# rayanirban/DiffSplitting

Measured on AMD Instinct MI355X. Metric: sampled images/sec (2000-step 128x128 SR3), higher is better.
Workload: dtype bf16; 1 GPU; sr_sr3_16_128: GaussianDiffusion.p_sample_loop, 16->128 SR3 UNet (97.8M params), T=2000 linear schedule; one step = UNet forward + posterior update of the batch; batch_per_gpu=16, global_batch=16, image=128x128x3, sample_steps=2000, parallelism=1 independent replicas, final RCCL all-gather, hipgraph=True, streams=1, noise=device Philox4x32-10, weights=random-init, seed 0

## Files before the change

### diffsplitting_amd/csrc/dsx_conv.hip

```cpp
#include "dsx_kernels.h"
#include <algorithm>
#include <cstdlib>
#include <mutex>
#include <type_traits>
#include <utility>

#ifndef DSX_WS_DEPTH_EXPR
#define DSX_WS_DEPTH_EXPR (bm == 64 ? 5 : (bm == 256 ? 2 : (ks == 1 ? 3 : 4)))
#endif
#ifndef DSX_PRE_RESID_EXPR
#define DSX_PRE_RESID_EXPR (NB == 1 && MB <= 2)
#endif
#ifndef DSX_PFF_EXPR
#define DSX_PFF_EXPR (NB == 2 ? 3 : 6)
#endif
#ifndef DSX_WS_K0_EXPR
#define DSX_WS_K0_EXPR 64
#endif
#ifndef DSX_EPI_PRIO_COND
#define DSX_EPI_PRIO_COND false
#endif
#ifndef DSX_STAMP_CVT_COND
#define DSX_STAMP_CVT_COND (tiC == 2 && gC == 0)
#endif
// ... 899 lines not shown
#pragma unroll
      for (int q = 0; q < 2 * NA; ++q) asm volatile("" : "+v"(av[q]));
#pragma unroll
      for (int it = 0; it < NIT; ++it) asm volatile("" : "+v"(rv[it]));
      DSX_STAMP_T(121, tid == 256 && DSX_STAMP_CVT_COND);
      float sc[CPU], sh[CPU];
#pragma unroll
      for (int q = 0; q < NA; ++q) {
        sc[4 * q] = gnF ? av[q].x : 1.0f; sc[4 * q + 1] = gnF ? av[q].y : 1.0f;
        sc[4 * q + 2] = gnF ? av[q].z : 1.0f; sc[4 * q + 3] = gnF ? av[q].w : 1.0f;
        sh[4 * q] = gnF ? av[NA + q].x : 0.0f; sh[4 * q + 1] = gnF ? av[NA + q].y : 0.0f;
        sh[4 * q + 2] = gnF ? av[NA + q].z : 0.0f; sh[4 * q + 3] = gnF ? av[NA + q].w : 0.0f;
      }
      const bool any_gn = a.gn_scale != nullptr;
      const bool plain = KS == 1 && !(gnF || a.swish);
      if (plain) {
#pragma unroll
        for (int it = 0; it < NIT; ++it) {
          if (loff[it] >= 0) {
            uint4 w = __builtin_bit_cast(uint4, rv[it]);
            const unsigned keep = ((edge[it] & flagsF) == 0 && cF < C) ? 0xffffffffu : 0u;
            w.x &= keep; w.y &= keep; w.z &= keep; w.w &= keep;
            lds_write_b128_asm(dst + loff[it], __builtin_bit_cast(f32x4_t, w));
          }
        }
      } else {
#pragma unroll
        for (int it = 0; it < NIT; ++it) {
          if (loff[it] >= 0) {
            float v[CPU];
            Unit<DT>::unpack(__builtin_bit_cast(uint4, rv[it]), v);
#ifndef DSX_ABL_CVT
            if (any_gn) affine_vec(v, sc, sh);
            if (a.swish) swish_vec(v);
#endif
            if (it == NIT - 1) { asm volatile("" :: "v"(v[0]), "v"(v[CPU - 1])); DSX_STAMP_T(122, tid == 256 && DSX_STAMP_CVT_COND); }
            uint4 w = Unit<DT>::pack(v);
            const unsigned keep = ((edge[it] & flagsF) == 0 && cF < C) ? 0xffffffffu : 0u;
            w.x &= keep; w.y &= keep; w.z &= keep; w.w &= keep;
            lds_write_b128_asm(dst + loff[it], __builtin_bit_cast(f32x4_t, w));
          }
        }
      }
      DSX_STAMP_T(123, tid == 256 && DSX_STAMP_CVT_COND);
    };
    auto wait_young = [&](int young) __attribute__((always_inline)) {
      if (young >= P) wait_vmcnt<P * NIT>();
      else if (P > 1 && young == P - 1) wait_vmcnt<(P > 1 ? (P - 1) * NIT : 0)>();
      else if (P > 2 && young == P - 2) wait_vmcnt<(P > 2 ? (P - 2) * NIT : 0)>();
      else if (P > 3 && young == P - 3) wait_vmcnt<(P > 3 ? (P - 3) * NIT : 0)>();
      else wait_vmcnt<0>();
      __builtin_amdgcn_sched_barrier(0);
    };

    int issued = 0, slotI = 0, slotF = 0;
    auto issue_next = [&]() __attribute__((always_inline)) {
      issue(slotI);
      ++issued;
      if (++slotI == NSLOT) slotI = 0;
    };
    auto fetch_next = [&]() __attribute__((always_inline)) {
      fetch(slotF);
      if (++slotF == NSLOT) slotF = 0;
    };
    DSX_STAMP_T(110, tid == 256);
    constexpr int K0 = DSX_WS_K0_EXPR < NSLOT ? DSX_WS_K0_EXPR : NSLOT;
    while (issued < K0 && issued < total) issue_next();
    DSX_STAMP_T(111, tid == 256);
    ws_barrier();
    wait_young(issued - 1);
    DSX_STAMP_T(112, tid == 256);
    fetch_next();
    for (int k = 0; k < 2 && issued < total && issued < NSLOT; ++k) issue_next();
    convert(0);
    if constexpr (NBUF >= 3) { if (total > 0) lds_signal(full_addr, wave, 1); }
    DSX_STAMP_T(113, tid == 256);
    if (total > 1) {
      wait_young(issued - 2);
      fetch_next();
    }
    if constexpr (NBUF == 2) ws_barrier();
    DSX_STAMP_T(64, tid == 256);
    int bufL = 1;
    for (int v = 0; v < total; ++v) {
      for (int k = 0; k < 2 && issued < total && issued < v + 1 + NSLOT; ++k) issue_next();
      DSX_STAMP_T(65 + 4 * v, tid == 256 && v < 9);
      if (v + 1 < total) {
        if constexpr (NBUF >= 3) {
          if (v + 1 >= NBUF) lds_wait_all_ge(full_addr + 16, v + 2 - NBUF, a.handoff_timeouts);
          convert(bufL);
          lds_signal(full_addr, wave, v + 2);
        } else {
          convert((v + 1) & 1);
        }
      }
      if (++bufL == NBUF) bufL = 0;
      DSX_STAMP_T(66 + 4 * v, tid == 256 && v < 9);
      if (v + 2 < total) {
        wait_young(issued - (v + 3));
        fetch_next();
      }
      DSX_STAMP_T(67 + 4 * v, tid == 256 && v < 9);
      if constexpr (NBUF == 2) ws_barrier();
      DSX_STAMP_T(68 + 4 * v, tid == 256 && v < 9);
    }
    return;
  }

  const int wm = wave / WN, wn = wave % WN;
  const int pq = ws16_pixel(c16);
  int abase[MB][KS];
#pragma unroll
  for (int mb = 0; mb < MB; ++mb) {
    const int m = (wm * MB + mb) * 32 + pq;
    const int tx = m & (TW - 1);
    const int ty = (m >> a.tw_log2) & (TH - 1);
    const int tb = m >> (a.tw_log2 + a.th_log2);
#pragma unroll
    for (int dy = 0; dy < KS; ++dy)
      abase[mb][dy] = (tb * PH + ty * S + dy) * RB + tx * S * PIXB + ws16_slice(kq) * 16;
  }
  const int a16 = TW >= 32 ? 16 * S * PIXB : (16 >> a.tw_log2) * S * RB;
  const int blk0 = (nt * WN + wn) * NB;
  const int wblock = G * (NSTEP * 1024);
  const __amdgpu_buffer_rsrc_t rsw = __builtin_amdgcn_make_buffer_rsrc(
      (void*)((const unsigned char*)a.wpack + (size_t)blk0 * wblock), 0, NB * wblock, 0x00020000);
  const int wlane[2] = {ws16_woff(lane, 0), ws16_woff(lane, 1)};
  static_assert(D % 2 == 0 && NSTEP % 2 == 0, "ring slots alternate between the two fragments of a pair");
  const int qtot = G * NSTEP;
  int qn = 0;
  struct WFrag { uint4 v[NB]; };
  auto load_b = [&](auto chc) __attribute__((always_inline)) -> WFrag {
    constexpr int ch = decltype(chc)::value;
    WFrag f;
#pragma unroll
    for (int nb = 0; nb < NB; ++nb)
      f.v[nb] = __builtin_bit_cast(uint4, __builtin_amdgcn_raw_buffer_load_b128(rsw, wlane[ch], nb * wblock + (qn >> 1) * 2048, 0));
    if (++qn == qtot) qn = 0;
    return f;
  };
  WFrag bq[D];
  static_for<D>([&](auto jc) __attribute__((always_inline)) {
    bq[decltype(jc)::value] = load_b(std::integral_constant<int, (decltype(jc)::value & 1)>{});
  });

  f32x16 acc[MB][NB];
#pragma unroll
  for (int mb = 0; mb < MB; ++mb)
#pragma unroll
    for (int nb = 0; nb < NB; ++nb)
#pragma unroll
      for (int r = 0; r < 16; ++r) acc[mb][nb][r] = 0.0f;

  const bool do_stats = a.stat_part != nullptr;
  const int nbase = blk0 * 32 + 8 * kq;

  struct TilePos { int tx, ty, b; };
  const int per_img = a.tiles_x * a.tiles_y;
  const int adv_x = a.ws_adv_x, adv_y = a.ws_adv_y, adv_b = a.ws_adv_b;
  auto tile_advance = [&](TilePos& t) __attribute__((always_inline)) {
    t.tx += adv_x;
    if (t.tx >= a.tiles_x) { t.tx -= a.tiles_x; t.ty += 1; }
    t.ty += adv_y;
    if (t.ty >= a.tiles_y) { t.ty -= a.tiles_y; t.b += 1; }
    t.b += adv_b;
  };
  int orow[MB], rrow[MB];
#pragma unroll
  for (int mb = 0; mb < MB; ++mb) {
    const int m = (wm * MB + mb) * 32 + pq;
    const int pix = (m >> a.tw_log2) * a.Wo + (m & (TW - 1));
    orow[mb] = pix * a.out_ld + nbase;
    rrow[mb] = pix * a.resid_ld + nbase;
  }
  const int p16 = TW >= 32 ? 16 : (16 >> a.tw_log2) * a.Wo;
  const int o16 = p16 * a.out_ld, r16 = p16 * a.resid_ld;
  auto tile_pixel0 = [&](const TilePos& t) __attribute__((always_inline)) -> int {
    return (t.b * a.Ho + (t.ty << a.th_log2)) * a.Wo + (t.tx << a.tw_log2);
  };
  TilePos cur;
  {
    const int q1 = (int)fastdiv((unsigned)p0, a.mg_tiles_x);
    cur.b = (int)fastdiv((unsigned)p0, a.mg_per_img);
    cur.tx = p0 - q1 * a.tiles_x;
    cur.ty = q1 - cur.b * a.tiles_y;
  }
  TilePos nxt = cur;
  tile_advance(nxt);
  TilePos nn = nxt;
  tile_advance(nn);

  auto load_aff = [&](int b, int slot) __attribute__((always_inline)) {
    if (a.gn_scale == nullptr || tid * 4 >= C) return;
    float* dst = aff_base + (size_t)slot * (AFFB / 4);
    *(float4*)(dst + tid * 4) = *(const float4*)(a.gn_scale + (size_t)b * C + tid * 4);
    *(float4*)(dst + C + tid * 4) = *(const float4*)(a.gn_shift + (size_t)b * C + tid * 4);
  };
  TilePos n3 = nn;
  tile_advance(n3);
  load_aff(cur.b, 0);
  if (ntile > 1) load_aff(nxt.b, 1);
  if (ntile > 2) load_aff(nn.b, 2);

  constexpr int NR = 8 / CPU;
  const float4 zero4 = make_float4(0.f, 0.f, 0.f, 0.f);
  float4 addv[NB][2], affv[2];
  constexpr bool PRE_RESID = DSX_PRE_RESID_EXPR;
  uint4 residv[PRE_RESID ? MB : 1][NB][2][NR];
#pragma unroll
  for (int nb = 0; nb < NB; ++nb)
#pragma unroll
    for (int j = 0; j < 2; ++j) addv[nb][j] = zero4;
  if (a.bias && !a.film) {
#pragma unroll
    for (int nb = 0; nb < NB; ++nb)
#pragma unroll
      for (int j = 0; j < 2; ++j) addv[nb][j] = *(const float4*)(a.bias + nbase + 32 * nb + 4 * j);
  }
#pragma unroll
  for (int mb = 0; mb < (PRE_RESID ? MB : 1); ++mb)
#pragma unroll
    for (int nb = 0; nb < NB; ++nb)
#pragma unroll
      for (int ph = 0; ph < 2; ++ph)
#pragma unroll
        for (int q = 0; q < NR; ++q) residv[mb][nb][ph][q] = make_uint4(0u, 0u, 0u, 0u);
  affv[0] = affv[1] = zero4;
  auto prefetch_epilogue = [&](const TilePos& t, bool want_aff, int b_aff) __attribute__((always_inline)) {
    if (a.film) {
#pragma unroll
      for (int nb = 0; nb < NB; ++nb)
#pragma unroll
        for (int j = 0; j < 2; ++j)
          addv[nb][j] = *(const float4*)(a.film + (size_t)t.b * a.film_bs + nbase + 32 * nb + 4 * j);
    }
    if (PRE_RESID && a.resid) {
      const int r0 = tile_pixel0(t) * a.resid_ld;
#pragma unroll
      for (int mb = 0; mb < (PRE_RESID ? MB : 1); ++mb)
#pragma unroll
        for (int ph = 0; ph < 2; ++ph) {
          const DT* rp = (const DT*)a.resid + (r0 + rrow[mb] + ph * r16);
#pragma unroll
          for (int nb = 0; nb < NB; ++nb)
#pragma unroll
            for (int q = 0; q < NR; ++q) residv[mb][nb][ph][q] = *(const uint4*)(rp + 32 * nb + CPU * q);
        }
    }
    if (want_aff && a.gn_scale != nullptr && tid * 4 < C) {
      affv[0] = *(const float4*)(a.gn_scale + (size_t)b_aff * C + tid * 4);
      affv[1] = *(const float4*)(a.gn_shift + (size_t)b_aff * C + tid * 4);
    }
  };
  prefetch_epilogue(cur, ntile > 3, n3.b);

  constexpr bool PF_OK = !(NB == 2 && KS == 3);
  unsigned fin_pf_acc = 0u;
  if constexpr (PF_OK) fin_pf_acc = l2_prefetch_fold(l2_prefetch(a.pf, blockIdx.x, gridDim.x, tid, 256));
  if constexpr (KS == 1) {
    if (a.fin_on) {
      fin_pf_acc |= l2_prefetch_fold(l2_prefetch(a.fin.pf, blockIdx.x, gridDim.x, tid, 256));
      const int nitems = a.fin.B * a.fin.groups;
      for (int item = (int)blockIdx.x * 4 + wave; item < nitems; item += (int)gridDim.x * 4)
        gn_finalize_item<1>(a.fin, item % a.fin.B, item / a.fin.B, lane, nullptr);
    }
  }

  if constexpr (NBUF >= 3) {
    if (tid < 8) ((unsigned*)(lds + NBUF * BUFB + 3 * AFFB + NSLOT * RAWB))[tid] = 0u;
  }
  ws_barrier();
  if constexpr (NBUF == 2) ws_barrier();
  DSX_STAMP_T(0, tid == 0);
  int g = 0, ti = 0, aslot = 0;
  int ibuf = 0;
  constexpr int NPAIR = NSTEP / 2;
  constexpr int NF = 2 * MB;
  constexpr int FT = NPAIR * NF;
  constexpr int PFF = (DSX_PFF_EXPR) < FT ? (DSX_PFF_EXPR) : FT - 1;
  static_assert(PFF >= 1 && PFF < FT && PFF <= 15, "lgkmcnt is 4 bits");
  constexpr int RP = D > NSTEP ? D / NSTEP : 1;
  if constexpr (RP == 1) {
    for (int v = 0; v < total; ++v) {
      constexpr int R0 = 0;
#define DSX_WS_ITEM_NEXT continue
#include "dsx_conv_ws_item.inc"
#undef DSX_WS_ITEM_NEXT
    }
  } else {
    for (int v0 = 0; v0 < total; v0 += RP)
      static_for<RP>([&](auto rc_) __attribute__((always_inline)) {
        constexpr int R0 = decltype(rc_)::value * NSTEP;
        const int v = v0 + decltype(rc_)::value;
        if (v >= total) return;
#define DSX_WS_ITEM_NEXT return
#include "dsx_conv_ws_item.inc"
#undef DSX_WS_ITEM_NEXT
      });
  }
  if constexpr (PF_OK) l2_prefetch_retire(a.pf, fin_pf_acc);
}


template <typename DT, int KS, int NPH>
__global__ __launch_bounds__(512, 1) void k_conv_img(const ConvArgs a) {
  constexpr int KC = Chunk<DT>::KC;
  constexpr int CPU = Unit<DT>::N;
  constexpr int ES = (int)sizeof(DT);
  constexpr int TAPS = KS * KS, PAD = KS / 2, PW = 8 + 2 * PAD;
  constexpr int PIXB = 80;
  constexpr int RB = KS == 3 ? 896 : 640;
  constexpr int IMGB = PW * RB;
  constexpr int NSTEP = TAPS * 2;
  constexpr int D = NSTEP;
  constexpr int MAXP = NPH;
  constexpr bool ALLW = NPH == 2;
  static_assert(NSTEP % D == 0, "ring depth divides the steps of a phase");
  extern __shared__ __attribute__((aligned(16))) unsigned char lds[];

  const int tid = threadIdx.x, lane = tid & 63;
  const int wave = __builtin_amdgcn_readfirstlane(tid >> 6);
  const int li = lane & 31, lh = lane >> 5;
  const int nb = blockIdx.x % a.nblocks, b = blockIdx.x / a.nblocks;
  const int C = a.C0 + a.C1;
  const int nphase = NPH != 8 ? NPH : C / (8 * KC);
  unsigned char* img = lds + wave * (2 * IMGB);
  float* aff = (float*)(lds + 8 * 2 * IMGB) + wave * (8 * 2 * KC);

  DSX_STAMP(0);
  if (KS == 3) {
    for (int q = lane; q < 360; q += 64) {
      const int bufi = q >= 180, r = q - 180 * bufi, bp = r / 5, u = r - 5 * bp;
      int py, px2;
      if (bp < 10) { py = 0; px2 = bp; }
      else if (bp < 20) { py = 9; px2 = bp - 10; }
      else { py = 1 + ((bp - 20) >> 1); px2 = ((bp - 20) & 1) ? 9 : 0; }
      *(uint4*)(img + bufi * IMGB + py * RB + px2 * PIXB + u * 16) = make_uint4(0u, 0u, 0u, 0u);
    }
  }

  auto load_raw = [&](int p, uint4 (&raw)[4]) __attribute__((always_inline)) {
    const int c0 = (p * 8 + wave) * KC;
    const bool first = c0 < a.C0;
    const char* src = (const char*)(first ? a.src0 : a.src1);
    const int Cs = first ? a.C0 : a.C1, cl = first ? c0 : c0 - a.C0;
#pragma unroll
    for (int i = 0; i < 4; ++i) {
      const int q = lane + 64 * i, px = q >> 2, u = q & 3;
      raw[i] = *(const uint4*)(src + (((size_t)b * 64 + px) * Cs + cl + u * CPU) * ES);
    }
  };
  auto convert_store = [&](int p, const uint4 (&raw)[4]) __attribute__((always_inline)) {
    unsigned char* buf = img + (p & 1) * IMGB;
    const int u = lane & 3;
    float sc[CPU], sh[CPU];
    if (a.has_gn) {
#pragma unroll
      for (int j = 0; j < CPU; ++j) { sc[j] = aff[p * 2 * KC + u * CPU + j]; sh[j] = aff[p * 2 * KC + KC + u * CPU + j]; }
    }
#pragma unroll
    for (int i = 0; i < 4; ++i) {
      const int px = (lane + 64 * i) >> 2;
      float v[CPU];
      Unit<DT>::unpack(raw[i], v);
      if (a.has_gn) affine_vec(v, sc, sh);
      if (a.swish) swish_vec(v);
      *(uint4*)(buf + ((px >> 3) + PAD) * RB + ((px & 7) + PAD) * PIXB + u * 16) = Unit<DT>::pack(v);
    }
  };

  uint2 glo[MAXP], ghi[MAXP];
  float gg[MAXP], gb[MAXP];
  if (a.has_gn) {
#pragma unroll
    for (int p = 0; p < MAXP; ++p) {
      const int pp = p < nphase ? p : nphase - 1;
      const int c0 = (pp * 8 + wave) * KC, cb = c0 & ~63, c = cb + lane;
      const bool first = cb < a.C0;
      const char* part = (const char*)(first ? a.gn_part0 : a.gn_part1);
      const int nch = first ? a.gn_nchunk0 : a.gn_nchunk1, pf32 = first ? a.gn_pf32_0 : a.gn_pf32_1;
      const int Cs = first ? a.C0 : a.C1, cl = first ? c : c - a.C0;
      const char* e = part + (((size_t)b * nch) * Cs + cl) * (pf32 ? 8 : 16);
      glo[p] = *(const uint2*)e;
      ghi[p] = *(const uint2*)(e + 8);
      gg[p] = a.gn_gamma[c]; gb[p] = a.gn_beta[c];
    }
  }
  uint4 raw0[4], raw1[4];
  load_raw(0, raw0);
  if (nphase > 1) load_raw(1, raw1);

  const unsigned char* wbase = (const unsigned char*)a.wpack + (size_t)nb * a.kchunks * (NSTEP * 1024) + lane * 16;
  int pn = 0, sn = 0;
  auto load_w = [&]() __attribute__((always_inline)) -> uint4 {
    const uint4 v = *(const uint4*)(wbase + ((size_t)(pn * 8 + wave) * NSTEP + sn) * 1024);
    if (++sn == NSTEP) { sn = 0; ++pn; }
    return v;
  };
  uint4 wq[D], wq1[ALLW ? D : 1];
#pragma unroll
  for (int j = 0; j < D; ++j) wq[j] = load_w();
  if constexpr (ALLW) {
    if (nphase > 1) {
#pragma unroll
      for (int j = 0; j < D; ++j) wq1[j] = load_w();
    }
  }
  DSX_STAMP(1);

  if (a.has_gn) {
    const int cpg = C / a.gn_groups;
    double gs[MAXP], gq[MAXP];
#pragma unroll
    for (int p = 0; p < MAXP; ++p) {
      const int pp = p < nphase ? p : nphase - 1;
      const int cb = ((pp * 8 + wave) * KC) & ~63, c = cb + lane;
      const bool first = cb < a.C0;
      const int nch = first ? a.gn_nchunk0 : a.gn_nchunk1, pf32 = first ? a.gn_pf32_0 : a.gn_pf32_1;
      const double d0 = __builtin_bit_cast(double, ((unsigned long long)glo[p].y << 32) | glo[p].x);
      const double d1 = __builtin_bit_cast(double, ((unsigned long long)ghi[p].y << 32) | ghi[p].x);
      gs[p] = pf32 ? (double)__builtin_bit_cast(float, glo[p].x) : d0;
      gq[p] = pf32 ? (double)__builtin_bit_cast(float, glo[p].y) : d1;
      if (nch > 1 && p < nphase) {
        const char* part = (const char*)(first ? a.gn_part0 : a.gn_part1);
        const int Cs = first ? a.C0 : a.C1, cl = first ? c : c - a.C0;
        for (int k = 1; k < nch; ++k) {
          const size_t idx = (((size_t)b * nch + k) * Cs + cl) * 2;
          if (pf32) { const float2 v = *(const float2*)((const float*)part + idx); gs[p] += v.x; gq[p] += v.y; }
          else { const double2 v = *(const double2*)((const double*)part + idx); gs[p] += v.x; gq[p] += v.y; }
        }
      }
      const StatPivot& piv = first ? a.gn_piv0 : a.gn_piv1;
      if (piv.bias || piv.film)
        stat_unshift(gs[p], gq[p], (double)stat_pivot(piv, b, first ? c : c - a.C0), (double)(a.Hs * a.Ws));
    }
    const float inv_n = 1.0f / (64.0f * (float)cpg);
#pragma unroll
    for (int p = 0; p < MAXP; ++p) {
      if (p < nphase) {
        const int c0 = (p * 8 + wave) * KC, c = (c0 & ~63) + lane;
        float s = (float)gs[p], q = (float)gq[p];
        for (int o = 1; o < cpg; o <<= 1) { s += __shfl_xor(s, o, 64); q += __shfl_xor(q, o, 64); }
        const double mean = (double)s * (double)inv_n;
        double var = (double)q * (double)inv_n - mean * mean;
        if (var < 0) var = 0;
        const float rstd = __builtin_amdgcn_rsqf((float)var + a.gn_eps);
        const float meanf = (float)mean;
        if (c >= c0 && c < c0 + KC) {
          const float sc = rstd * gg[p];
          aff[p * 2 * KC + (c - c0)] = sc;
          aff[p * 2 * KC + KC + (c - c0)] = gb[p] - meanf * sc;
        }
      }
    }
  }
  const PfAcc pf_acc = l2_prefetch(a.pf, blockIdx.x, gridDim.x, tid, 512);
  DSX_STAMP(2);
  __builtin_amdgcn_s_waitcnt(0xC07F);
  convert_store(0, raw0);
  if (nphase > 1) convert_store(1, raw1);
  DSX_STAMP(3);

  int abase[2][KS];
#pragma unroll
  for (int mb = 0; mb < 2; ++mb) {
    const int m = mb * 32 + li;
#pragma unroll
    for (int dy = 0; dy < KS; ++dy) abase[mb][dy] = ((m >> 3) + dy) * RB + (m & 7) * PIXB + lh * 16;
  }
  f32x16 acc[2];
#pragma unroll
  for (int mb = 0; mb < 2; ++mb)
#pragma unroll
    for (int r = 0; r < 16; ++r) acc[mb][r] = 0.f;

  for (int p = 0; p < nphase; ++p) {
    const unsigned char* buf = img + (p & 1) * IMGB;
    if (p + 2 < nphase) load_raw(p + 2, raw0);
    const bool more = p + 1 < nphase;
    static_for<NSTEP>([&](auto sc_) __attribute__((always_inline)) {
      constexpr int s = decltype(sc_)::value;
      constexpr int tap = s >> 1, fs = s & 1, dy = tap / KS, dx = tap % KS;
      uint4 wcur = wq[s % D];
      if constexpr (ALLW) {
        if (p == 1) wcur = wq1[s % D];
      } else {
        if (more) wq[s % D] = load_w();
      }
#pragma unroll
      for (int mb = 0; mb < 2; ++mb) {
        const f32x4_t px = *(const f32x4_t*)(buf + abase[mb][dy] + dx * PIXB + fs * 32);
        acc[mb] = mfma_step<DT>(wcur, px, acc[mb]);
      }
    });
    if (p + 2 < nphase) convert_store(p + 2, raw0);
    DSX_STAMP(4 + p);
  }

  const int px = tid >> 3, cg = (tid & 7) * 4;
  const int n0 = nb * 32 + cg;
  const size_t opix = (size_t)b * 64 + px;
  float4 eb = make_float4(0.f, 0.f, 0.f, 0.f), ef = eb;
  float er[4] = {0.f, 0.f, 0.f, 0.f};
  if (a.bias) eb = *(const float4*)(a.bias + n0);
  if (a.film) ef = *(const float4*)(a.film + (size_t)b * a.film_bs + n0);
  if (a.resid) {
#pragma unroll
    for (int j = 0; j < 4; ++j) er[j] = act_load<DT>(a.resid, opix * a.resid_ld + n0 + j);
  }
  __syncthreads();
  DSX_STAMP(12);
  float* part = (float*)lds;
#pragma unroll
  for (int mb = 0; mb < 2; ++mb)
#pragma unroll
    for (int j = 0; j < 4; ++j)
      *(float4*)(part + ((wave * 2 + mb) * 64 + lane) * 20 + 4 * j) =
          make_float4(acc[mb][4 * j], acc[mb][4 * j + 1], acc[mb][4 * j + 2], acc[mb][4 * j + 3]);
  __syncthreads();
  DSX_STAMP(13);
  const int mbo = px >> 5, lo = (px & 31) + 32 * (cg >> 4), r0 = cg & 15;
  float x[4] = {0.f, 0.f, 0.f, 0.f};
#pragma unroll
  for (int w = 0; w < 8; ++w) {
    const float4 t = *(const float4*)(part + ((w * 2 + mbo) * 64 + lo) * 20 + r0);
    x[0] += t.x; x[1] += t.y; x[2] += t.z; x[3] += t.w;
  }
  x[0] += eb.x; x[1] += eb.y; x[2] += eb.z; x[3] += eb.w;
  x[0] += ef.x; x[1] += ef.y; x[2] += ef.z; x[3] += ef.w;
#pragma unroll
  for (int j = 0; j < 4; ++j) x[j] += er[j];
  const int okind = a.out_bf16;
  if (okind == 0) {
    *(float4*)((float*)a.out + opix * a.out_ld + n0) = make_float4(x[0], x[1], x[2], x[3]);
  } else {
    uint2 w2;
    if (okind == 1) { w2.x = pack_bf16x2(x[0], x[1]); w2.y = pack_bf16x2(x[2], x[3]); }
    else { w2.x = pack_f16x2(x[0], x[1]); w2.y = pack_f16x2(x[2], x[3]); }
    *(uint2*)((unsigned short*)a.out + opix * a.out_ld + n0) = w2;
  }
  DSX_STAMP(14);
  if (a.stat_part != nullptr) {
    float s1[4], s2[4];
#pragma unroll
    for (int j = 0; j < 4; ++j) { s1[j] = x[j]; s2[j] = x[j] * x[j]; }
#pragma unroll
    for (int o = 8; o < 64; o <<= 1)
#pragma unroll
      for (int j = 0; j < 4; ++j) { s1[j] += __shfl_xor(s1[j], o, 64); s2[j] += __shfl_xor(s2[j], o, 64); }
    __syncthreads();
    float* red = (float*)lds;
    if (lane < 8) {
#pragma unroll
      for (int j = 0; j < 4; ++j) { red[(wave * 32 + cg + j) * 2] = s1[j]; red[(wave * 32 + cg + j) * 2 + 1] = s2[j]; }
    }
    __syncthreads();
    if (tid < 64) {
      const int ch = tid >> 1, k = tid & 1;
      float t = 0.f;
#pragma unroll
      for (int w = 0; w < 8; ++w) t += red[(w * 32 + ch) * 2 + k];
      a.stat_part[((size_t)b * a.Cout + nb * 32 + ch) * 2 + k] = t;
    }
  }
  l2_prefetch_retire(a.pf, pf_acc);
  DSX_STAMP(15);
}

static size_t conv_img_lds(int dtype, int ks) {
  const int KC = dtype != 0 ? 32 : 16;
  const int pw = ks == 3 ? 10 : 8, rb = ks == 3 ? 896 : 640;
  return (size_t)8 * 2 * pw * rb + (size_t)8 * 8 * 2 * KC * sizeof(float);
}
bool conv_img_applicable(int dtype, int ks, int stride, const ConvArgs& a, bool gn, int gn_groups) {
  if (stride != 1 || a.up || !(ks == 1 || ks == 3)) return false;
  if (a.Hs != 8 || a.Ws != 8 || a.Ho != 8 || a.Wo != 8) return false;
  const int KC = dtype != 0 ? 32 : 16, C = a.C0 + a.C1;
  if (a.C0 % (8 * KC) || a.C1 % (8 * KC) || C / (8 * KC) > 8 || C < 8 * KC) return false;
  if (a.Cout % 32 || (a.out_ld & 3) || (a.resid && (a.resid_ld & 3))) return false;
  if (gn) {
    if (gn_groups < 1 || C % gn_groups) return false;
    const int cpg = C / gn_groups;
    if (cpg > 64 || (cpg & (cpg - 1)) || a.C0 % cpg) return false;
  }
  return true;
}


template <typename DT>
__global__ __launch_bounds__(256) void k_conv_first(const ConvArgs a) {
  constexpr bool F32 = sizeof(DT) == 4;
  constexpr int ES = (int)sizeof(DT);
  constexpr int KSTEP = F32 ? 2 : 16;
  constexpr int NS16 = 4;
  __shared__ __attribute__((aligned(16))) unsigned char sm[18 * 18 * 7 * 4 + 64 * 4];
  DT* patch = (DT*)sm;
  int* kofft = (int*)(sm + 18 * 18 * 7 * 4);

  const int tid = threadIdx.x, lane = tid & 63;
  const int wave = __builtin_amdgcn_readfirstlane(tid >> 6);
  const int li = lane & 31, lh = lane >> 5;
  const int Cin = a.C0 + a.C1, K = 9 * Cin;
  const int tiles_x = a.Wo >> 4, tiles_y = a.Ho >> 4;
  const int t = blockIdx.x % (tiles_x * tiles_y), b = blockIdx.x / (tiles_x * tiles_y);
  const int ty = t / tiles_x, tx = t - ty * tiles_x;
  const int oy0 = ty * 16, ox0 = tx * 16;
  const int NBLK = (a.Cout + 31) >> 5;

  for (int e = tid; e < 18 * 18 * Cin; e += 256) {
    const int c = e % Cin, pp = e / Cin, px = pp % 18, py = pp / 18;
    const int iy = oy0 + py - 1, ix = ox0 + px - 1;
    DT v = (DT)0.f;
    if (iy >= 0 && iy < a.Hs && ix >= 0 && ix < a.Ws) {
      const size_t pix = ((size_t)b * a.Hs + iy) * a.Ws + ix;
      v = c < a.C0 ? ((const DT*)a.src0)[pix * a.C0 + c] : ((const DT*)a.src1)[pix * a.C1 + (c - a.C0)];
    }
    patch[e] = v;
  }
  if (F32 && tid < 64) {
    const int k = tid < K ? tid : 0;
    const int tap = k / Cin, c = k - tap * Cin;
    kofft[tid] = ((tap / 3) * 18 + (tap % 3)) * Cin + c;
  }
  int koff[F32 ? 1 : NS16 * 8];
  if constexpr (!F32) {
#pragma unroll
    for (int s = 0; s < NS16; ++s)
#pragma unroll
      for (int j = 0; j < 8; ++j) {
        int k = 16 * s + 8 * lh + j;
        if (k >= K) k = 0;
        const int tap = k / Cin, c = k - tap * Cin;
        koff[s * 8 + j] = (((tap / 3) * 18 + (tap % 3)) * Cin + c) * 2;
      }
  }
  uint4 wf[F32 ? 1 : 2 * NS16];
  if constexpr (!F32) {
#pragma unroll
    for (int nb = 0; nb < 2; ++nb)
#pragma unroll
      for (int s = 0; s < NS16; ++s)
        wf[nb * NS16 + s] = nb < NBLK ? ((const uint4*)a.wpack)[(nb * NS16 + s) * 64 + lane] : make_uint4(0u, 0u, 0u, 0u);
  }
  __syncthreads();

  f32x16 acc[2][2];
#pragma unroll
  for (int mb = 0; mb < 2; ++mb)
#pragma unroll
    for (int nb = 0; nb < 2; ++nb)
#pragma unroll
      for (int r = 0; r < 16; ++r) acc[mb][nb][r] = 0.f;

#pragma unroll
  for (int mb = 0; mb < 2; ++mb) {
    const int m = (wave * 2 + mb) * 32 + li;
    const int base = ((m >> 4) * 18 + (m & 15)) * Cin;
    if constexpr (F32) {
      const int nsteps = (K + 1) >> 1;
      const float* wp = (const float*)a.wpack;
      for (int s = 0; s < nsteps; ++s) {
        const float pv = ((const float*)patch)[base + kofft[2 * s + lh]];
#pragma unroll
        for (int nb = 0; nb < 2; ++nb) {
          if (nb < NBLK) acc[mb][nb] = __builtin_amdgcn_mfma_f32_32x32x2f32(wp[(nb * 32 + s) * 64 + lane], pv, acc[mb][nb], 0, 0, 0);
        }
      }
    } else {
      const unsigned char* pb = (const unsigned char*)patch + base * 2;
#pragma unroll
      for (int s = 0; s < NS16; ++s) {
        unsigned w4[4];
#pragma unroll
        for (int q = 0; q < 4; ++q) {
          const unsigned lo = *(const unsigned short*)(pb + koff[s * 8 + 2 * q]);
          const unsigned hi = *(const unsigned short*)(pb + koff[s * 8 + 2 * q + 1]);
          w4[q] = lo | (hi << 16);
        }
        const f32x4_t px = __builtin_bit_cast(f32x4_t, make_uint4(w4[0], w4[1], w4[2], w4[3]));
#pragma unroll
        for (int nb = 0; nb < 2; ++nb)
          if (nb < NBLK) acc[mb][nb] = mfma_step<DT>(wf[nb * NS16 + s], px, acc[mb][nb]);
      }
    }
  }
  (void)KSTEP; (void)ES;

  const int okind = a.out_bf16;
#pragma unroll
  for (int nb = 0; nb < 2; ++nb) {
    const int nbase = nb * 32 + 16 * lh;
    if (nb >= NBLK) continue;
    float s1[16], s2[16];
#pragma unroll
    for (int r = 0; r < 16; ++r) { s1[r] = 0.f; s2[r] = 0.f; }
    const bool live = nbase < a.Cout;
#pragma unroll
    for (int mb = 0; mb < 2; ++mb) {
      const int m = (wave * 2 + mb) * 32 + li;
      const size_t opix = ((size_t)b * a.Ho + (oy0 + (m >> 4))) * a.Wo + (ox0 + (m & 15));
      float x[16], pv[16];
#pragma unroll
      for (int r = 0; r < 16; ++r) { x[r] = acc[mb][nb][r]; pv[r] = 0.f; }
      if (live) {
        if (a.bias) {
#pragma unroll
          for (int j = 0; j < 4; ++j) { const float4 tt = *(const float4*)(a.bias + nbase + 4 * j); pv[4 * j] = tt.x; pv[4 * j + 1] = tt.y; pv[4 * j + 2] = tt.z; pv[4 * j + 3] = tt.w; }
#pragma unroll
          for (int r = 0; r < 16; ++r) x[r] += pv[r];
        }
        store16<true>(a.out, opix * a.out_ld + nbase, x, okind, 16);
#pragma unroll
        for (int r = 0; r < 16; ++r) { const float d = x[r] - pv[r]; s1[r] += d; s2[r] += d * d; }
      }
    }
    if (a.stat_part != nullptr) {
      float w1 = row16_fold(s1, lane), w2 = row16_fold(s2, lane);
      w1 += __shfl_xor(w1, 16, 64);
      w2 += __shfl_xor(w2, 16, 64);
      const int nch = tiles_x * tiles_y * 4, chunk = t * 4 + wave;
      const int n = nbase + row16_fold_reg(li);
      if (li < 16 && n < a.Cout) {
        float* pp = a.stat_part + (((size_t)b * nch + chunk) * a.Cout + n) * 2;
        pp[0] = w1; pp[1] = w2;
      }
    }
  }
}

bool conv_first_applicable(int ks, int stride, const ConvArgs& a, bool gn) {
  const int C = a.C0 + a.C1;
  return ks == 3 && stride == 1 && !a.up && !gn && !a.swish && C >= 1 && C <= 7 && a.Cout >= 16 && a.Cout <= 64 &&
         (a.Cout & 15) == 0 && (a.Ho & 15) == 0 && (a.Wo & 15) == 0 && a.Ho == a.Hs && a.Wo == a.Ws && a.out_ld == a.Cout;
}
hipError_t launch_conv_first(int dtype, const ConvArgs& a, hipStream_t st) {
  const unsigned grid = (unsigned)(a.B * (a.Ho >> 4) * (a.Wo >> 4));
  if (dtype == 1) hipLaunchKernelGGL(k_conv_first<__bf16>, dim3(grid), dim3(256), 0, st, a);
  else if (dtype == 2) hipLaunchKernelGGL(k_conv_first<_Float16>, dim3(grid), dim3(256), 0, st, a);
  else hipLaunchKernelGGL(k_conv_first<float>, dim3(grid), dim3(256), 0, st, a);
  return hipGetLastError();
}

enum ConvFamily { FAM_MFMA, FAM_WS, FAM_IMG };
struct ConvVariant {
  int family, dtype, tile, ks, stride, cpg;
  void (*kern)(const ConvArgs);
  int block, lds_cap;
  int MB, WM, WN, NB;
  int max_px;
  int nit;
  int depth, nbuf;
  bool fuses_stats;
};
static constexpr int kLdsDefault = 64 * 1024, kLdsMax = 160 * 1024;
static constexpr int conv_cpg(int ks) { return ks == 1 ? 2 : 1; }
int conv_chunk_multiple(int ks) { return conv_cpg(ks); }

static constexpr int mfma_max_px(int bm, int ks, int stride, int cpg) {
  if (ks == 1) return bm;
  if (stride == 2) return 400;
  if (cpg == 2) return bm == 256 ? 324 : 220;
  return bm == 256 ? 400 : (bm == 128 ? 220 : 144);
}
template <typename DT, int TILE, int MB, int WM, int WN, int KS, int S = 1, int CPG = conv_cpg(KS)>
constexpr ConvVariant mfma_row() {
  constexpr bool G2 = KS == 3 && CPG == 2;
  constexpr int D = KS == 1 ? 4 : (G2 ? 6 : DSX_RING_DEPTH);
  constexpr int PX = mfma_max_px(32 * MB * WM, KS, S, CPG);
  constexpr int MI = (PX * 4 * CPG + 255) / 256;
  return {FAM_MFMA, Kind<DT>::value, TILE, KS, S, CPG, k_conv_mfma<DT, MB, WM, WN, KS, S, CPG, D, MI>, 256,
          G2 ? kLdsMax : kLdsDefault, MB, WM, WN, 1, PX, MI, 0, 2, MB <= 2};
}

static constexpr int kWsLoaderWaves = 4;
static constexpr int ws_max_px(int bm, int ks) { return ks == 1 ? bm : (bm == 256 ? 324 : (bm == 128 ? 180 : 108)); }
static constexpr int ws_depth(int bm, int ks, int cpg) {
#ifndef DSX_WS_DEPTH_C2_64
#define DSX_WS_DEPTH_C2_64 3
#endif
  if (ks == 3 && cpg == 2) return bm == 64 ? DSX_WS_DEPTH_C2_64 : 2;
  if (ks == 3 && cpg == 4) return 1;
  if (ks == 1 && cpg == 4) return bm == 64 ? 2 : 1;
  return DSX_WS_DEPTH_EXPR;
}
template <typename DT, int TILE, int MB, int WM, int WN, int NB, int KS, int CPG = conv_cpg(KS)>
constexpr ConvVariant ws_row() {
  constexpr int BM = 32 * MB * WM;
  constexpr int D = KS == 1 ? ((NB == 2 || MB == 4) ? DSX_RING_1X1_NB2 : DSX_RING_1X1_NB1) : ((NB == 2 || MB == 4) ? 6 : 18);
  constexpr int PX = ws_max_px(BM, KS);
  constexpr int NIT = (PX * 4 * CPG + kWsLoaderWaves * 64 - 1) / (kWsLoaderWaves * 64);
  constexpr int P = ws_depth(BM, KS, CPG);
  return {FAM_WS, Kind<DT>::value, TILE, KS, 1, CPG, k_conv_ws<DT, MB, WM, WN, NB, KS, CPG, D, NIT, P, kWsLoaderWaves>,
          256 + 64 * kWsLoaderWaves, kLdsMax, MB, WM, WN, NB, PX, NIT, P, ws_nbuf(BM, KS, NB, CPG), true};
}

template <typename DT, int KS, int NPH> constexpr ConvVariant img_row() {
  return {FAM_IMG, Kind<DT>::value, -1, KS, 1, NPH, k_conv_img<DT, KS, NPH>, 512, kLdsMax, 0, 0, 0, 0, 0, 0, 0, 0, true};
}

template <int N> struct ConvVariants {
  ConvVariant row[N];
  constexpr const ConvVariant* begin() const { return row; }
  constexpr const ConvVariant* end() const { return row + N; }
};
template <int... N> constexpr ConvVariants<(N + ...)> concat(const ConvVariants<N>&... parts) {
  ConvVariants<(N + ...)> out{};
  int n = 0;
  auto append = [&](const auto& p) { for (const ConvVariant& v : p) out.row[n++] = v; };
  (append(parts), ...);
  return out;
}

template <typename DT> constexpr ConvVariants<34> variants_of() {
  return {{
      mfma_row<DT, TILE_256x128, 8, 1, 4, 1>(), mfma_row<DT, TILE_256x128, 8, 1, 4, 3>(),
      mfma_row<DT, TILE_128x128, 4, 1, 4, 1>(), mfma_row<DT, TILE_128x128, 4, 1, 4, 3>(),
      mfma_row<DT, TILE_64x128, 2, 1, 4, 1>(), mfma_row<DT, TILE_64x128, 2, 1, 4, 3>(),
      mfma_row<DT, TILE_256x64, 4, 2, 2, 1>(), mfma_row<DT, TILE_256x64, 4, 2, 2, 3>(),
      mfma_row<DT, TILE_128x64, 2, 2, 2, 1>(), mfma_row<DT, TILE_128x64, 2, 2, 2, 3>(),
      mfma_row<DT, TILE_128x64, 2, 2, 2, 3, 1, 2>(),
      mfma_row<DT, TILE_64x64, 1, 2, 2, 1>(), mfma_row<DT, TILE_64x64, 1, 2, 2, 3>(),
      mfma_row<DT, TILE_64x64, 1, 2, 2, 3, 2>(),
      mfma_row<DT, TILE_128x32, 1, 4, 1, 1>(), mfma_row<DT, TILE_128x32, 1, 4, 1, 3>(),
      mfma_row<DT, TILE_128x32, 1, 4, 1, 3, 1, 2>(), mfma_row<DT, TILE_256x32, 2, 4, 1, 3, 1, 2>(),
      ws_row<DT, TILE_64x128, 2, 1, 4, 1, 1>(), ws_row<DT, TILE_64x128, 2, 1, 4, 1, 3>(),
      ws_row<DT, TILE_64x128, 2, 1, 4, 1, 1, 4>(),
      ws_row<DT, TILE_64x128, 2, 1, 4, 1, 3, 2>(),
      ws_row<DT, TILE_64x128, 2, 1, 4, 1, 3, 4>(),
      ws_row<DT, TILE_128x64, 2, 2, 2, 1, 1>(), ws_row<DT, TILE_128x64, 2, 2, 2, 1, 3>(),
      ws_row<DT, TILE_256x64, 4, 2, 2, 1, 3>(),
      ws_row<DT, TILE_64x64, 1, 2, 2, 1, 1>(), ws_row<DT, TILE_64x64, 1, 2, 2, 1, 3>(),
      img_row<DT, 1, 2>(), img_row<DT, 1, 4>(), img_row<DT, 1, 8>(),
      img_row<DT, 3, 2>(), img_row<DT, 3, 4>(), img_row<DT, 3, 8>(),
  }};
}
template <typename DT> constexpr ConvVariants<4> ws_nb2_variants() {
  return {{ws_row<DT, TILE_128x128, 2, 2, 2, 2, 1>(), ws_row<DT, TILE_128x128, 2, 2, 2, 2, 3>(),
           ws_row<DT, TILE_128x128, 2, 2, 2, 2, 1, 4>(), ws_row<DT, TILE_128x128, 2, 2, 2, 2, 3, 2>()}};
}
static constexpr auto kVariants = concat(variants_of<float>(), variants_of<__bf16>(), variants_of<_Float16>(),
                                         ws_nb2_variants<__bf16>(), ws_nb2_variants<_Float16>());

static constexpr int kKeySlots = 3 * 3 * (TILE_COUNT + 1) * 2 * 2 * 4;
static constexpr int key_slot(int family, int dtype, int tile, int ks, int stride, int cpg) {
  const int c = cpg == 1 ? 0 : (cpg == 2 ? 1 : (cpg == 4 ? 2 : (cpg == 8 ? 3 : -1)));
  if (family < 0 || family > FAM_IMG || dtype < 0 || dtype > 2 || tile < -1 || tile >= TILE_COUNT || (ks != 1 && ks != 3) ||
      (stride != 1 && stride != 2) || c < 0)
    return -1;
  return ((((family * 3 + dtype) * (TILE_COUNT + 1) + tile + 1) * 2 + ks / 2) * 2 + stride - 1) * 4 + c;
}
struct VariantIndex { short row[kKeySlots]; bool unique; };
static constexpr VariantIndex index_variants() {
  VariantIndex ix{};
  for (short& r : ix.row) r = -1;
  ix.unique = true;
  short n = 0;
  for (const ConvVariant& v : kVariants) {
    const int s = key_slot(v.family, v.dtype, v.tile, v.ks, v.stride, v.cpg);
    if (s < 0 || ix.row[s] >= 0) ix.unique = false;
    else ix.row[s] = n;
    ++n;
  }
  return ix;
}
static constexpr VariantIndex kIndex = index_variants();
static_assert(kIndex.unique, "kVariants: two rows share a key, or a key is outside key_slot's ranges");
static const ConvVariant* find_variant(int family, int dtype, int tile, int ks, int stride, int cpg) {
  const int s = key_slot(family, dtype, tile, ks, stride, cpg);
  return s >= 0 && kIndex.row[s] >= 0 ? &kVariants.row[kIndex.row[s]] : nullptr;
// ... 188 lines not shown
```

Measured before the change: 2.797 images/s.

## Interleave weight prefetch and next-phase conversion into 8x8 conv prologue and MFMA loop

Restructures the k_conv_img kernel for 8x8 images. Weight loads are spread across the GroupNorm-stat prologue in scheduled slices instead of issued up front, dropping the special all-weights path for two phases. Conversion of the next phase's activations into LDS is folded into the MFMA step loop, and the raw buffers ping-pong between phases. It also adds timestamp stamps on two threads. The aim is to hide global-load latency and prologue work behind compute, at the cost of higher register pressure and more scheduling constraints.

Measured after the change: 2.833 images/s (median of 6 runs). 1.01x the previous value.

```diff
diff --git a/diffsplitting_amd/csrc/dsx_conv.hip b/diffsplitting_amd/csrc/dsx_conv.hip
--- a/diffsplitting_amd/csrc/dsx_conv.hip
+++ b/diffsplitting_amd/csrc/dsx_conv.hip
@@ -1225,6 +1225,7 @@
 }
 
 
+#define IMG_STAMP(i) do { DSX_STAMP_T((i), tid == 0); DSX_STAMP_T(32 + (i), tid == 448); } while (0)
 template <typename DT, int KS, int NPH>
 __global__ __launch_bounds__(512, 1) void k_conv_img(const ConvArgs a) {
   constexpr int KC = Chunk<DT>::KC;
@@ -1237,8 +1238,10 @@
   constexpr int NSTEP = TAPS * 2;
   constexpr int D = NSTEP;
   constexpr int MAXP = NPH;
-  constexpr bool ALLW = NPH == 2;
   static_assert(NSTEP % D == 0, "ring depth divides the steps of a phase");
+  constexpr int WTOP0 = D < 4 ? D : 4;
+  constexpr int WREST = D - WTOP0;
+  constexpr int WSLOTS = 2 * MAXP + 4;
   extern __shared__ __attribute__((aligned(16))) unsigned char lds[];
 
   const int tid = threadIdx.x, lane = tid & 63;
@@ -1250,7 +1253,7 @@
   unsigned char* img = lds + wave * (2 * IMGB);
   float* aff = (float*)(lds + 8 * 2 * IMGB) + wave * (8 * 2 * KC);
 
-  DSX_STAMP(0);
+  IMG_STAMP(0);
   if (KS == 3) {
     for (int q = lane; q < 360; q += 64) {
       const int bufi = q >= 180, r = q - 180 * bufi, bp = r / 5, u = r - 5 * bp;
@@ -1273,23 +1276,21 @@
       raw[i] = *(const uint4*)(src + (((size_t)b * 64 + px) * Cs + cl + u * CPU) * ES);
     }
   };
-  auto convert_store = [&](int p, const uint4 (&raw)[4]) __attribute__((always_inline)) {
+  auto convert_prep = [&](int p, float (&sc)[CPU], float (&sh)[CPU]) __attribute__((always_inline)) {
+    const int u = lane & 3;
+    if (a.has_gn) {
+#pragma unroll
+      for (int j = 0; j < CPU; ++j) { sc[j] = aff[p * 2 * KC + u * CPU + j]; sh[j] = aff[p * 2 * KC + KC + u * CPU + j]; }
+    }
+  };
+  auto convert_unit = [&](int p, const uint4& raw, int i, const float (&sc)[CPU], const float (&sh)[CPU]) __attribute__((always_inline)) {
     unsigned char* buf = img + (p & 1) * IMGB;
-    const int u = lane & 3;
-    float sc[CPU], sh[CPU];
-    if (a.has_gn) {
-#pragma unroll
-      for (int j = 0; j < CPU; ++j) { sc[j] = aff[p * 2 * KC + u * CPU + j]; sh[j] = aff[p * 2 * KC + KC + u * CPU + j]; }
-    }
-#pragma unroll
-    for (int i = 0; i < 4; ++i) {
-      const int px = (lane + 64 * i) >> 2;
-      float v[CPU];
-      Unit<DT>::unpack(raw[i], v);
-      if (a.has_gn) affine_vec(v, sc, sh);
-      if (a.swish) swish_vec(v);
-      *(uint4*)(buf + ((px >> 3) + PAD) * RB + ((px & 7) + PAD) * PIXB + u * 16) = Unit<DT>::pack(v);
-    }
+    const int u = lane & 3, px = (lane + 64 * i) >> 2;
+    float v[CPU];
+    Unit<DT>::unpack(raw, v);
+    if (a.has_gn) affine_vec(v, sc, sh);
+    if (a.swish) swish_vec(v);
+    *(uint4*)(buf + ((px >> 3) + PAD) * RB + ((px & 7) + PAD) * PIXB + u * 16) = Unit<DT>::pack(v);
   };
 
   uint2 glo[MAXP], ghi[MAXP];
@@ -1311,7 +1312,6 @@
   }
   uint4 raw0[4], raw1[4];
   load_raw(0, raw0);
-  if (nphase > 1) load_raw(1, raw1);
 
   const unsigned char* wbase = (const unsigned char*)a.wpack + (size_t)nb * a.kchunks * (NSTEP * 1024) + lane * 16;
   int pn = 0, sn = 0;
@@ -1320,22 +1320,23 @@
     if (++sn == NSTEP) { sn = 0; ++pn; }
     return v;
   };
-  uint4 wq[D], wq1[ALLW ? D : 1];
-#pragma unroll
-  for (int j = 0; j < D; ++j) wq[j] = load_w();
-  if constexpr (ALLW) {
-    if (nphase > 1) {
-#pragma unroll
-      for (int j = 0; j < D; ++j) wq1[j] = load_w();
-    }
-  }
-  DSX_STAMP(1);
-
-  if (a.has_gn) {
-    const int cpg = C / a.gn_groups;
-    double gs[MAXP], gq[MAXP];
-#pragma unroll
-    for (int p = 0; p < MAXP; ++p) {
+  uint4 wq[D];
+  auto issue_w = [&](auto g_) __attribute__((always_inline)) {
+    constexpr int G = decltype(g_)::value;
+    constexpr int lo = G < 0 ? 0 : WTOP0 + WREST * G / WSLOTS, hi = G < 0 ? WTOP0 : WTOP0 + WREST * (G + 1) / WSLOTS;
+    __builtin_amdgcn_sched_barrier(0);
+    static_for<hi - lo>([&](auto j_) __attribute__((always_inline)) {
+      wq[lo + decltype(j_)::value] = load_w();
+    });
+    __builtin_amdgcn_sched_barrier(0);
+  };
+  issue_w(std::integral_constant<int, -1>{});
+  IMG_STAMP(1);
+
+  double gs[MAXP], gq[MAXP];
+  static_for<MAXP>([&](auto p_) __attribute__((always_inline)) {
+    constexpr int p = decltype(p_)::value;
+    if (a.has_gn) {
       const int pp = p < nphase ? p : nphase - 1;
       const int cb = ((pp * 8 + wave) * KC) & ~63, c = cb + lane;
       const bool first = cb < a.C0;
@@ -1344,6 +1345,9 @@
       const double d1 = __builtin_bit_cast(double, ((unsigned long long)ghi[p].y << 32) | ghi[p].x);
       gs[p] = pf32 ? (double)__builtin_bit_cast(float, glo[p].x) : d0;
       gq[p] = pf32 ? (double)__builtin_bit_cast(float, glo[p].y) : d1;
+#ifdef DSX_STAMPS
+      if constexpr (p == 0) { asm volatile("" :: "v"(gs[0]), "v"(gq[0])); IMG_STAMP(19); }
+#endif
       if (nch > 1 && p < nphase) {
         const char* part = (const char*)(first ? a.gn_part0 : a.gn_part1);
         const int Cs = first ? a.C0 : a.C1, cl = first ? c : c - a.C0;
@@ -1357,10 +1361,15 @@
       if (piv.bias || piv.film)
         stat_unshift(gs[p], gq[p], (double)stat_pivot(piv, b, first ? c : c - a.C0), (double)(a.Hs * a.Ws));
     }
+    issue_w(std::integral_constant<int, p>{});
+    if constexpr (p == 0) { if (nphase > 1) load_raw(1, raw1); }
+  });
+  {
+    const int cpg = a.has_gn ? C / a.gn_groups : 1;
     const float inv_n = 1.0f / (64.0f * (float)cpg);
-#pragma unroll
-    for (int p = 0; p < MAXP; ++p) {
-      if (p < nphase) {
+    static_for<MAXP>([&](auto p_) __attribute__((always_inline)) {
+      constexpr int p = decltype(p_)::value;
+      if (a.has_gn && p < nphase) {
         const int c0 = (p * 8 + wave) * KC, c = (c0 & ~63) + lane;
         float s = (float)gs[p], q = (float)gq[p];
         for (int o = 1; o < cpg; o <<= 1) { s += __shfl_xor(s, o, 64); q += __shfl_xor(q, o, 64); }
@@ -1375,14 +1384,22 @@
           aff[p * 2 * KC + KC + (c - c0)] = gb[p] - meanf * sc;
         }
       }
-    }
+      issue_w(std::integral_constant<int, MAXP + p>{});
+    });
+  }
+  IMG_STAMP(2);
+  __builtin_amdgcn_s_waitcnt(0xC07F);
+  {
+    float sc[CPU], sh[CPU];
+    convert_prep(0, sc, sh);
+    static_for<4>([&](auto i_) __attribute__((always_inline)) {
+      constexpr int i = decltype(i_)::value;
+      convert_unit(0, raw0[i], i, sc, sh);
+      issue_w(std::integral_constant<int, 2 * MAXP + i>{});
+    });
   }
   const PfAcc pf_acc = l2_prefetch(a.pf, blockIdx.x, gridDim.x, tid, 512);
-  DSX_STAMP(2);
-  __builtin_amdgcn_s_waitcnt(0xC07F);
-  convert_store(0, raw0);
-  if (nphase > 1) convert_store(1, raw1);
-  DSX_STAMP(3);
+  IMG_STAMP(3);
 
   int abase[2][KS];
 #pragma unroll
@@ -1397,27 +1414,45 @@
 #pragma unroll
     for (int r = 0; r < 16; ++r) acc[mb][r] = 0.f;
 
-  for (int p = 0; p < nphase; ++p) {
+  auto phase = [&](int p, uint4 (&rnext)[4], const uint4 (&rcvt)[4]) __attribute__((always_inline)) {
     const unsigned char* buf = img + (p & 1) * IMGB;
-    if (p + 2 < nphase) load_raw(p + 2, raw0);
+#ifdef DSX_STAMPS
+    if (p == nphase - 1) { asm volatile("s_waitcnt vmcnt(0)" ::: "memory"); IMG_STAMP(16); }
+#endif
+    if (p + 2 < nphase) load_raw(p + 2, rnext);
     const bool more = p + 1 < nphase;
+    float csc[CPU], csh[CPU];
+    if (more) convert_prep(p + 1, csc, csh);
     static_for<NSTEP>([&](auto sc_) __attribute__((always_inline)) {
       constexpr int s = decltype(sc_)::value;
       constexpr int tap = s >> 1, fs = s & 1, dy = tap / KS, dx = tap % KS;
-      uint4 wcur = wq[s % D];
-      if constexpr (ALLW) {
-        if (p == 1) wcur = wq1[s % D];
-      } else {
-        if (more) wq[s % D] = load_w();
-      }
+      const uint4 wcur = wq[s % D];
+      if (more) wq[s % D] = load_w();
 #pragma unroll
       for (int mb = 0; mb < 2; ++mb) {
         const f32x4_t px = *(const f32x4_t*)(buf + abase[mb][dy] + dx * PIXB + fs * 32);
         acc[mb] = mfma_step<DT>(wcur, px, acc[mb]);
       }
+      if constexpr (s == 0) { if (p == 0) IMG_STAMP(18); }
+      static_for<4 * (s + 1) / NSTEP - 4 * s / NSTEP>([&](auto i_) __attribute__((always_inline)) {
+        constexpr int i = 4 * s / NSTEP + decltype(i_)::value;
+        if (more) convert_unit(p + 1, rcvt[i], i, csc, csh);
+      });
     });
-    if (p + 2 < nphase) convert_store(p + 2, raw0);
-    DSX_STAMP(4 + p);
+    if (p == 0) IMG_STAMP(17);
+    IMG_STAMP(4 + p);
+  };
+  if constexpr (NPH != 8) {
+    static_for<NPH / 2>([&](auto h_) __attribute__((always_inline)) {
+      constexpr int p = 2 * decltype(h_)::value;
+      phase(p, raw0, raw1);
+      phase(p + 1, raw1, raw0);
+    });
+  } else {
+    for (int p = 0; p < nphase; p += 2) {
+      phase(p, raw0, raw1);
+      if (p + 1 < nphase) phase(p + 1, raw1, raw0);
+    }
   }
 
   const int px = tid >> 3, cg = (tid & 7) * 4;
@@ -1431,8 +1466,9 @@
 #pragma unroll
     for (int j = 0; j < 4; ++j) er[j] = act_load<DT>(a.resid, opix * a.resid_ld + n0 + j);
   }
+  IMG_STAMP(20);
   __syncthreads();
-  DSX_STAMP(12);
+  IMG_STAMP(12);
   float* part = (float*)lds;
 #pragma unroll
   for (int mb = 0; mb < 2; ++mb)
@@ -1441,7 +1477,7 @@
       *(float4*)(part + ((wave * 2 + mb) * 64 + lane) * 20 + 4 * j) =
           make_float4(acc[mb][4 * j], acc[mb][4 * j + 1], acc[mb][4 * j + 2], acc[mb][4 * j + 3]);
   __syncthreads();
-  DSX_STAMP(13);
+  IMG_STAMP(13);
   const int mbo = px >> 5, lo = (px & 31) + 32 * (cg >> 4), r0 = cg & 15;
   float x[4] = {0.f, 0.f, 0.f, 0.f};
 #pragma unroll
@@ -1462,7 +1498,7 @@
     else { w2.x = pack_f16x2(x[0], x[1]); w2.y = pack_f16x2(x[2], x[3]); }
     *(uint2*)((unsigned short*)a.out + opix * a.out_ld + n0) = w2;
   }
-  DSX_STAMP(14);
+  IMG_STAMP(14);
   if (a.stat_part != nullptr) {
     float s1[4], s2[4];
 #pragma unroll
@@ -1487,7 +1523,7 @@
     }
   }
   l2_prefetch_retire(a.pf, pf_acc);
-  DSX_STAMP(15);
+  IMG_STAMP(15);
 }
 
 static size_t conv_img_lds(int dtype, int ks) {
```
